# microsoft/Sora

Hardware: NVIDIA B200
Metric: 802.11a RX PHY Msamples/s (IQ in, bits out) (higher is better)
Workload: dtype int16 (fixed point; uint8 path metrics)

## Files before the change

sora_b200/csrc/fixed.cuh:

```cuda
#pragma once
#include <stdint.h>
#include <cuda_runtime.h>

namespace sb {

struct cs16 { int re, im; };

__host__ __device__ __forceinline__ int sx16(int v) { return (int)(short)v; }
__host__ __device__ __forceinline__ int sat16(int v) { return v > 32767 ? 32767 : (v < -32768 ? -32768 : v); }
__host__ __device__ __forceinline__ int wadd(int a, int b) { return (int)((unsigned)a + (unsigned)b); }

__host__ __device__ __forceinline__ cs16 unpack(uint32_t w) { cs16 c; c.re = (int)(short)(w & 0xFFFF); c.im = (int)w >> 16; return c; }
__host__ __device__ __forceinline__ uint32_t pack(cs16 c) { return ((uint32_t)c.re & 0xFFFFu) | ((uint32_t)c.im << 16); }
__host__ __device__ __forceinline__ cs16 mk(int re, int im) { cs16 c; c.re = re; c.im = im; return c; }

__host__ __device__ __forceinline__ cs16 sra(cs16 a, int n) { return mk(a.re >> n, a.im >> n); }
__host__ __device__ __forceinline__ cs16 adds(cs16 a, cs16 b) { return mk(sat16(a.re + b.re), sat16(a.im + b.im)); }
__host__ __device__ __forceinline__ cs16 subs(cs16 a, cs16 b) { return mk(sat16(a.re - b.re), sat16(a.im - b.im)); }
__host__ __device__ __forceinline__ cs16 subw(cs16 a, cs16 b) { return mk(sx16(a.re - b.re), sx16(a.im - b.im)); }
__host__ __device__ __forceinline__ cs16 cnot(cs16 a) { return mk(~a.re, ~a.im); }
__host__ __device__ __forceinline__ int neg16(int v) { return sx16(-v); }

__host__ __device__ __forceinline__ void cmul_conj32(int& re, int& im, cs16 a, cs16 b) {
    re = wadd(a.re * b.re, a.im * b.im);
    im = wadd(neg16(b.im) * a.re, b.re * a.im);
}
__host__ __device__ __forceinline__ void cmul32(int& re, int& im, cs16 a, cs16 b) {
    re = wadd(a.re * b.re, a.im * neg16(b.im));
    im = wadd(a.re * b.im, a.im * b.re);
}
__host__ __device__ __forceinline__ cs16 cmul_q15(cs16 a, cs16 b) {
    int re, im; cmul32(re, im, a, b); return mk(sx16(re >> 15), sx16(im >> 15));
}
__host__ __device__ __forceinline__ cs16 cmul_tw(cs16 a, cs16 w) {
    int re = wadd(a.re * w.re, a.im * (int)(short)~w.im);
    int im = wadd(a.re * w.im, a.im * w.re);
    return mk(sx16(re >> 15), sx16(im >> 15));
}
__host__ __device__ __forceinline__ cs16 mulj(cs16 a) { return mk(~a.im, a.re); }

__host__ __device__ __forceinline__ void r4_butterfly(cs16& a, cs16& b, cs16& c, cs16& d, cs16 w1, cs16 w2, cs16 w3) {
    a = sra(a, 2); b = sra(b, 2); c = sra(c, 2); d = sra(d, 2);
    cs16 ac = adds(a, c), bd = adds(b, d), a_c = subs(a, c), b_d = subs(b, d);
    cs16 jbd = mulj(b_d);
    a = adds(ac, bd);
    b = cmul_tw(subs(ac, bd), w2);
    c = cmul_tw(subs(a_c, jbd), w1);
    d = cmul_tw(adds(a_c, jbd), w3);
}
__host__ __device__ __forceinline__ void dft4(cs16& v0, cs16& v1, cs16& v2, cs16& v3) {
    cs16 x0 = sra(v0, 2), x1 = sra(v1, 2), x2 = sra(v2, 2), x3 = sra(v3, 2);
    cs16 s0 = adds(x0, x2), s1 = adds(x1, x3), s2 = adds(cnot(x2), x0), s3 = adds(cnot(x3), x1);
    cs16 t3 = mk(s3.im, ~s3.re);
    v0 = adds(s0, s1); v1 = adds(cnot(s1), s0); v2 = adds(s2, t3); v3 = adds(cnot(t3), s2);
}

}
```

sora_b200/csrc/rx11a_kernels.cuh:

```cuda
#pragma once
#include "tables.cuh"
#include "viterbi_k7_common.cuh"

namespace sb {

__device__ __forceinline__ int d_uatan2(const DevTables& T, int y, int x) {
    unsigned ay = y > 0 ? (unsigned)y : 0u - (unsigned)y, ax = x > 0 ? (unsigned)x : 0u - (unsigned)x;
    int ys = ay > 1 ? 31 - __clz(ay) : 0, xs = ax > 1 ? 31 - __clz(ax) : 0;
    int shift = max(xs, ys) - 6;
    if (shift > 0) { y >>= shift; x >>= shift; }
    return (int)__ldg(&T.atan2_lut[((unsigned)y & 0xFF) * 256 + ((unsigned)x & 0xFF)]);
}
__device__ __forceinline__ cs16 d_rot(const DevTables& T, int th) {
    return unpack(__ldg(T.rot + ((unsigned)th & 0xFFFFu)));
}

struct CcaState {
    uint32_t his[4][4];
    int acr[4], aci[4], eng[4];
    int his_idx, acc_i, acr_reg, aci_reg, eng_reg;
    unsigned auto_count, sense_count, high_count; int sync_state, peak_corr, peak_index;
    unsigned dc_cnt; int dc_sum_re, dc_sum_im;
    __device__ void reset() {
        for (int i = 0; i < 4; i++) { for (int j = 0; j < 4; j++) his[i][j] = 0; acr[i] = aci[i] = eng[i] = 0; }
// ... 113 lines not shown
        r4_butterfly(a, b, c, d, unpack(__ldg(T.tw64 + lane)), unpack(__ldg(T.tw64 + 16 + lane)), unpack(__ldg(T.tw64 + 32 + lane)));
        x[lane] = pack(a); x[lane + 16] = pack(b); x[lane + 32] = pack(c); x[lane + 48] = pack(d);
    }
    __syncwarp();
    if (lane < 16) {
        int base = (lane >> 2) * 16, fidx = lane & 3;
        cs16 a = unpack(x[base + fidx]), b = unpack(x[base + fidx + 4]), c = unpack(x[base + fidx + 8]), d = unpack(x[base + fidx + 12]);
        r4_butterfly(a, b, c, d, unpack(__ldg(T.tw16 + fidx)), unpack(__ldg(T.tw16 + 4 + fidx)), unpack(__ldg(T.tw16 + 8 + fidx)));
        x[base + fidx] = pack(a); x[base + fidx + 4] = pack(b); x[base + fidx + 8] = pack(c); x[base + fidx + 12] = pack(d);
    }
    __syncwarp();
    if (lane < 16) {
        cs16 a = unpack(x[4 * lane]), b = unpack(x[4 * lane + 1]), c = unpack(x[4 * lane + 2]), d = unpack(x[4 * lane + 3]);
        dft4(a, b, c, d);
        x[4 * lane] = pack(a); x[4 * lane + 1] = pack(b); x[4 * lane + 2] = pack(c); x[4 * lane + 3] = pack(d);
    }
    __syncwarp();
}
__device__ __forceinline__ int bitrev6(int i) { return (int)(__brev((unsigned)i) >> 26); }

__device__ __forceinline__ uint32_t warp_viterbi_signal(const uint8_t* soft, int lane) {
    const unsigned FULL = 0xFFFFFFFFu;
    const int cA = ((lane >> 1) ^ (lane >> 2) ^ (lane >> 4)) & 1;
    const int cB = (lane ^ (lane >> 1) ^ (lane >> 2)) & 1;
    int m0 = lane == 0 ? 0x00 : 0x30, m1 = 0x30;
    uint32_t decE[24], decO[24];
#pragma unroll
    for (int t = 0; t < 24; t++) {
        int tA = 2 * soft[2 * t], tB = 2 * soft[2 * t + 1];
        int alpha = (cA ? 14 - tA : tA) + (cB ? 14 - tB : tB), beta = 28 - alpha;
        int n0 = min((m0 + alpha) & 0xFE, ((m1 + beta) & 0xFF) | 1);
        int n1 = min((m0 + beta) & 0xFE, ((m1 + alpha) & 0xFF) | 1);
        decE[t] = __ballot_sync(FULL, n0 & 1); decO[t] = __ballot_sync(FULL, n1 & 1);
        int w = n0 | (n1 << 8);
        int wa = __shfl_sync(FULL, w, lane >> 1), wb = __shfl_sync(FULL, w, 16 + (lane >> 1));
        int sh = 8 * (lane & 1);
        m0 = (wa >> sh) & 0xFF; m1 = (wb >> sh) & 0xFF;
        if (((t + 1) & 7) == 0) {
            int mn = __reduce_min_sync(FULL, min(m0, m1)) & 0xFE;
            m0 = (m0 - mn) & 0xFF; m1 = (m1 - mn) & 0xFF;
        }
    }
    unsigned key = min(((unsigned)m0 << 8) | ((unsigned)lane << 2), ((unsigned)m1 << 8) | ((unsigned)(lane + 32) << 2));
    key = __reduce_min_sync(FULL, key);
    int pos = (int)(key >> 2) & 0x7F;
    uint32_t word = 0;
#pragma unroll
    for (int i = 0; i < 24; i++) {
        word |= (uint32_t)((pos >> 6) & 1) << (23 - i);
        pos = (pos >> 1) & 0x3F;
        int col = 23 - i;
        int bit = 0;
        if (col >= 1) { uint32_t wsel = (pos & 1) ? decO[col - 1] : decE[col - 1]; bit = (wsel >> (pos >> 1)) & 1; }
        pos |= bit << 6;
    }
    return word >> 6;
}

struct FrontTaps {
    uint32_t* freq_coeffs; uint32_t* chan_coeffs; uint32_t* fft_out; uint32_t* equalized; uint32_t* tracked; uint32_t max_sym;
    uint32_t hdr_only;
};

__device__ __forceinline__ int data_index(int bin) {
    if (bin >= 38) { if (bin == 43 || bin == 57) return -1; return bin - 38 - (bin > 43) - (bin > 57); }
    if (bin >= 1 && bin <= 26) { if (bin == 7 || bin == 21) return -1; return 24 + bin - 1 - (bin > 7) - (bin > 21); }
    return -1;
}

#define SB_FRONT_WARPS 4
#ifndef SB_FRONT_MINB
#define SB_FRONT_MINB 6
#endif
template <int STAGE>
__global__ void __launch_bounds__(32 * SB_FRONT_WARPS, SB_FRONT_MINB) k_front11a(const uint32_t* __restrict__ iq, const uint64_t* __restrict__ off,
        const uint32_t* __restrict__ len, uint32_t nframes, DevTables T, FrameInfo* __restrict__ info,
        uint8_t* __restrict__ soft_out, uint64_t soft_stride, const uint16_t* __restrict__ inv_deint, FrontTaps taps, uint32_t sh, uint32_t lsh) {
    __shared__ uint32_t s_fft[SB_FRONT_WARPS][2][64];
    __shared__ __align__(16) uint8_t s_soft[SB_FRONT_WARPS][288];
    __shared__ uint32_t s_demap[256];
    __shared__ uint8_t s_pilot[128];
    __shared__ __align__(16) uint32_t s_stage[STAGE == 2 ? SB_FRONT_WARPS : 1][2][STAGE == 2 ? 328 : 4];
    __shared__ __align__(8) unsigned long long s_mbar[STAGE == 2 ? SB_FRONT_WARPS : 1][2];
    const unsigned FULL = 0xFFFFFFFFu;
    const int lane = threadIdx.x & 31, wib = threadIdx.x >> 5;
    if (STAGE == 2 && lane == 0) {
        asm volatile("mbarrier.init.shared::cta.b64 [%0], 1;" :: "r"((uint32_t)__cvta_generic_to_shared(&s_mbar[wib][0])));
        asm volatile("mbarrier.init.shared::cta.b64 [%0], 1;" :: "r"((uint32_t)__cvta_generic_to_shared(&s_mbar[wib][1])));
        asm volatile("fence.mbarrier_init.release.cluster;" ::: "memory");
    }
    for (int i = threadIdx.x; i < 256; i += blockDim.x)
        s_demap[i] = (uint32_t)__ldg(T.demap + i) | ((uint32_t)__ldg(T.demap + 256 + i) << 8) | ((uint32_t)__ldg(T.demap + 512 + i) << 16) | ((uint32_t)__ldg(T.demap + 768 + i) << 24);
    for (int i = threadIdx.x; i < 128; i += blockDim.x) s_pilot[i] = __ldg(T.pilot_neg + i);
    __syncthreads();
    const uint32_t f = blockIdx.x * SB_FRONT_WARPS + wib;
    if (f >= nframes) return;
    FrameInfo fi = info[f];
    if (fi.status != E_SUCCESS) return;
    uint8_t* sb = s_soft[wib];
    const uint32_t* x = iq + off[f];
    const uint32_t nvec = ((len[f] << lsh) / 28u) * 28u / 8u;
    const uint32_t s0 = fi.detect_vec * 4u;
    if (fi.detect_vec + 36u > nvec) { if (lane == 0) info[f].status = E_NO_FRAME; return; }
    const int half = lane >> 4, hl = lane & 15;
    const int b0 = lane, b1 = lane + 32;
    const int r0 = bitrev6(b0), r1 = bitrev6(b1);
// ... 174 lines not shown
            const uint32_t mb = (uint32_t)__cvta_generic_to_shared(&s_mbar[wib][b]), dst = (uint32_t)__cvta_generic_to_shared(&s_stage[wib][b][0]);
            asm volatile("mbarrier.arrive.expect_tx.shared::cta.b64 _, [%0], %1;" :: "r"(mb), "r"(bytes) : "memory");
            asm volatile("cp.async.bulk.shared::cluster.global.mbarrier::complete_tx::bytes [%0], [%1], %2, [%3];" :: "r"(dst), "l"(a0), "r"(bytes), "r"(mb) : "memory");
        }
    };
    auto stage_wait = [&](int b) {
        if (st_cnt[b] == 0) return;
        const uint32_t mb = (uint32_t)__cvta_generic_to_shared(&s_mbar[wib][b]); uint32_t ok = 0;
        while (!ok) asm volatile("{ .reg .pred p; mbarrier.try_wait.parity.shared::cta.b64 p, [%1], %2; selp.u32 %0, 1, 0, p; }" : "=r"(ok) : "r"(mb), "r"(st_par[b]) : "memory");
        st_par[b] ^= 1u;
    };
    auto stage_load4 = [&](int b, uint32_t first, cs16 (&v)[4]) {
        const uint32_t skew = (uint32_t)(((uintptr_t)(x + (st_base[b] << sh)) & 15u) >> 2);
#pragma unroll
        for (int j = 0; j < 4; j++) v[j] = cmul_q15(sra(unpack(s_stage[wib][b][skew + ((first - st_base[b] + hl + 16u * j) << sh)]), 1), fcv[j]);
    };
    if (STAGE == 2 && more) stage_issue(0, s0 + 144u + 80u, 160u);
    if (STAGE == 1 && more) prefetch_regs(s0 + 144u + 80u * (1u + (uint32_t)half) + 8u);
    for (uint32_t sym = 1; more; sym += 2) {
        const bool haveA = sym_ready(sym), haveB = remain >= 2 && sym_ready(sym + 1);
        if (!haveA) { status = E_NO_FRAME; break; }
        {   cs16 v[4];
            const uint32_t mine = (half && haveB) ? sym + 1 : sym;
            const uint32_t first = s0 + 144u + 80u * mine + 8u;
            if (STAGE == 2) {
                const int b = (int)(st_i & 1u);
                const bool staged = st_base[b] == s0 + 144u + 80u * sym && st_cnt[b] >= (mine - sym + 1u) * 80u;
                stage_wait(b);
                if (staged) stage_load4(b, first, v); else load4(first, v);
                __syncwarp();
                st_i++; stage_issue((int)(st_i & 1u), s0 + 144u + 80u * (sym + 2u), 160u);
            } else if (STAGE == 1) {
                if (raw_first == first) {
#pragma unroll
                    for (int j = 0; j < 4; j++) v[j] = cmul_q15(sra(unpack(raw[j]), 1), fcv[j]);
                } else load4(first, v);
                prefetch_regs(s0 + 144u + 80u * (sym + 2u + (uint32_t)half) + 8u);
            } else load4(first, v);
            fft_from_regs(v[0], v[1], v[2], v[3]); }
        more = post_fft(0, sym);
        if (!more) break;
        if (!haveB) {
            if (remain >= 1 && !sym_ready(sym + 1)) { status = E_NO_FRAME; break; }
            sym -= 1;
            if (STAGE == 2) { stage_wait((int)(st_i & 1u)); __syncwarp(); stage_issue((int)(st_i & 1u), s0 + 144u + 80u * (sym + 2u), 160u); }
            continue;
        }
        more = post_fft(1, sym + 1);
    }
    if (STAGE == 2) { stage_wait((int)(st_i & 1u)); __syncwarp(); }
    if (lane == 0) { fi.status = status; fi.soft_bytes = soft_bytes; info[f] = fi; }
}

__host__ __device__ inline uint32_t resampled_len_40(uint32_t len44) {
    const uint32_t n = len44 / 28u * 28u, q = n / 11u, rem = n % 11u;
    const uint32_t m = 10u * q + (rem >= 1u ? 1u : 0u) + (rem > 2u ? rem - 2u : 0u);
    return m / 28u * 28u;
}
__global__ void __launch_bounds__(256) k_resample_44_40(const uint32_t* __restrict__ iq, const uint64_t* __restrict__ off, const uint32_t* __restrict__ len,
                                                        uint32_t nframes, uint32_t* __restrict__ out, uint64_t out_stride ,
                                                        uint64_t* __restrict__ off40, uint32_t* __restrict__ len40) {
    const uint32_t f = blockIdx.x;
    if (f >= nframes) return;
    const uint32_t n40 = resampled_len_40(len[f]);
    if (blockIdx.y == 0 && threadIdx.x == 0) { off40[f] = (uint64_t)f * out_stride; len40[f] = n40; }
    const uint32_t* x = iq + off[f];
    uint32_t* y = out + (size_t)f * out_stride;
    for (uint32_t m = blockIdx.y * blockDim.x + threadIdx.x; m < n40; m += gridDim.y * blockDim.x) {
        const uint32_t k = m / 10u, r = m - 10u * k;
        if (r == 0) { y[m] = __ldg(x + 11u * k); continue; }
        const int R = r == 1 ? 115 : r == 2 ? 102 : r == 3 ? 90 : r == 4 ? 77 : r == 5 ? 64 : r == 6 ? 51 : r == 7 ? 38 : r == 8 ? 26 : 13;
        const int L = r == 1 ? 13 : r == 2 ? 26 : r == 3 ? 38 : r == 4 ? 51 : r == 5 ? 64 : r == 6 ? 77 : r == 7 ? 90 : r == 8 ? 102 : 115;
        const cs16 a = unpack(__ldg(x + 11u * k + r)), b = unpack(__ldg(x + 11u * k + r + 1u));
        y[m] = pack(mk(sx16((a.re * R + b.re * L) >> 7), sx16((a.im * R + b.im * L) >> 7)));
    }
}

}
```

sora_b200/csrc/sb200.cu:

```cuda
#include "../../include/sora_b200.h"
#include "viterbi_k7_re.cuh"
#include "viterbi_k7_lane.cuh"
#include "rx11b_kernels.cuh"
#include "rx11n_kernels.cuh"
#include "tx11a_kernels.cuh"
#include "tx11b_kernels.cuh"
#include "tx11b_legacy_kernels.cuh"
#include "tx11n_kernels.cuh"
#include "fir_kernels.cuh"
#include <stdlib.h>
#include <string>
#include <vector>
#include <chrono>
#include <string.h>
#include <new>
#include <stdio.h>
#include <thread>
#include <mutex>
#include <condition_variable>
#include <atomic>
#include <emmintrin.h>

using namespace sb;

// ... 293 lines not shown
            if (r[1]) return h->fail(SB200_E_INVALID, "slot exceeds iq_total_samples");
            h->tab_max_len = r[0]; h->tab_host = need_host_copy;
            if (h->tab_immutable) { h->tab_off = frame_off; h->tab_len = frame_len; h->tab_n = nframes; h->tab_total = iq_total; }
        }
        *d_off = frame_off; *d_len = frame_len; *max_len = h->tab_max_len; *host_valid = h->tab_host && (cached || need_host_copy);
        return SB200_OK;
    }
    h->tab_off = nullptr;
    offh.resize(nframes); lenh.resize(nframes);
    if (off_dev) CK(cudaMemcpyAsync(offh.data(), frame_off, nframes * 8ull, cudaMemcpyDeviceToHost, st)); else memcpy(offh.data(), frame_off, nframes * 8ull);
    if (len_dev) CK(cudaMemcpyAsync(lenh.data(), frame_len, nframes * 4ull, cudaMemcpyDeviceToHost, st)); else memcpy(lenh.data(), frame_len, nframes * 4ull);
    if (off_dev || len_dev) CK(cudaStreamSynchronize(st));
    uint32_t mx = 0;
    for (uint32_t i = 0; i < nframes; i++) {
        if (lenh[i] > iq_total || offh[i] > iq_total - lenh[i]) return h->fail(SB200_E_INVALID, "slot exceeds iq_total_samples");
        if (lenh[i] > mx) mx = lenh[i];
    }
    if (off_dev) *d_off = frame_off; else { CK(h->off.need(nframes * 8ull)); CK(cudaMemcpyAsync(h->off.p, offh.data(), nframes * 8ull, cudaMemcpyHostToDevice, st)); *d_off = (const uint64_t*)h->off.p; }
    if (len_dev) *d_len = frame_len; else { CK(h->len.need(nframes * 4ull)); CK(cudaMemcpyAsync(h->len.p, lenh.data(), nframes * 4ull, cudaMemcpyHostToDevice, st)); *d_len = (const uint32_t*)h->len.p; }
    *max_len = mx; *host_valid = true;
    return SB200_OK;
}

static cudaError_t vring_need(sb200_handle* h, uint32_t n) {
    if (n >= h->lane_min) return h->vring.need((size_t)((n + SB_VL_FR - 1) / SB_VL_FR) * SB_VL_NB8D * SB_VL_ENTRY * 16);
    return cudaSuccess;
}
template <int CR>
static void launch_viterbi_re(sb200_handle* h, uint32_t n, cudaStream_t s, const uint8_t* soft, uint64_t soft_stride, const uint32_t* list, const uint32_t* cnt,
                              const FrameInfo* info, const VitJob& job, uint8_t* out, uint64_t out_stride, uint32_t raw_off, uint32_t* nraw) {
    const unsigned g = (n + SB_VR_FR - 1) / SB_VR_FR, gp = (n + 15) / 16;
    uint4* const ring = (uint4*)h->vring.p;
    h->last_vit = n >= h->lane_min ? "k_viterbi_lane" : "k_viterbi_re";
    if (n >= h->lane_min && h->vl_hb == 8 && h->vl_defer) k_viterbi_lane<CR, 8, true><<<(n + SB_VL_FR - 1) / SB_VL_FR, 32, h->vl_pad_smem, s>>>(soft, soft_stride, n, list, cnt, info, job, out, out_stride, raw_off, nraw, ring, h->vl_flags);
    else if (n >= h->lane_min && h->vl_hb == 8) k_viterbi_lane<CR, 8><<<(n + SB_VL_FR - 1) / SB_VL_FR, 32, h->vl_pad_smem, s>>>(soft, soft_stride, n, list, cnt, info, job, out, out_stride, raw_off, nraw, ring, h->vl_flags);
    else if (n >= h->lane_min)       k_viterbi_lane<CR, 6><<<(n + SB_VL_FR - 1) / SB_VL_FR, 32, h->vl_pad_smem, s>>>(soft, soft_stride, n, list, cnt, info, job, out, out_stride, raw_off, nraw, ring, h->vl_flags);
    else if (h->use_pair)            k_viterbi_re<CR, 1><<<gp, 32, 0, s>>>(soft, soft_stride, n, list, cnt, info, job, out, out_stride, raw_off, nraw);
    else                             k_viterbi_re<CR, 2><<<g, 32, 0, s>>>(soft, soft_stride, n, list, cnt, info, job, out, out_stride, raw_off, nraw);
}

static int launch_chunk(sb200_handle* h, const uint32_t* iq_base, const uint64_t* d_off, const uint32_t* d_len, uint32_t f0, uint32_t f1,
                        uint64_t soft_stride, uint64_t row, cudaStream_t sf, cudaStream_t sv, cudaEvent_t front_done, FrontTaps taps, bool timed, const int2* dc_init = nullptr, uint32_t chunk_idx = 0, uint32_t sh = 1, uint32_t lsh = 0) {
    const uint32_t n = f1 - f0;
    FrameInfo* d_info = (FrameInfo*)h->info.p + f0;
    uint8_t* d_soft = (uint8_t*)h->soft.p + (size_t)f0 * soft_stride;
    uint8_t* d_out = (uint8_t*)h->out.p + (size_t)f0 * row;
    uint32_t* d_status = (uint32_t*)h->status.p + f0; uint32_t* d_crc = (uint32_t*)h->crc.p + f0;
    if (timed) CK(cudaEventRecord(h->evk[0], sf));
    k_sync11a<<<(n + 127) / 128, 128, 0, sf>>>(iq_base, d_off + f0, d_len + f0, n, h->cca_thr, h->T, d_info, dc_init ? dc_init + f0 : nullptr, sh, lsh);
    if (timed) CK(cudaEventRecord(h->evk[1], sf));
    {   const dim3 g((n + SB_FRONT_WARPS - 1) / SB_FRONT_WARPS), b(32 * SB_FRONT_WARPS);
        if (h->front_stage == 2) k_front11a<2><<<g, b, 0, sf>>>(iq_base, d_off + f0, d_len + f0, n, h->T, d_info, d_soft, soft_stride, h->inv_deint, taps, sh, lsh);
        else if (h->front_stage == 1) k_front11a<1><<<g, b, 0, sf>>>(iq_base, d_off + f0, d_len + f0, n, h->T, d_info, d_soft, soft_stride, h->inv_deint, taps, sh, lsh);
        else k_front11a<0><<<g, b, 0, sf>>>(iq_base, d_off + f0, d_len + f0, n, h->T, d_info, d_soft, soft_stride, h->inv_deint, taps, sh, lsh); }
    if (timed) CK(cudaEventRecord(h->evk[2], sf));
    if (sv != sf) { CK(cudaEventRecord(front_done, sf)); CK(cudaStreamWaitEvent(sv, front_done, 0)); }
    VitJob job{}; job.depth = 256; job.lookahead = 24; job.raw = 0;
    if (h->use_v2) {
        const unsigned g = (n + SB_VQ_FR - 1) / SB_VQ_FR, b = 32 * SB_VQ_WARPS;
        k_viterbi_quad<CR_34><<<g, b, h->vq_pad_smem, sv>>>(d_soft, soft_stride, n, d_info, job, h->T, d_out, row, d_status, d_crc);
        k_viterbi_quad<CR_12><<<g, b, 0, sv>>>(d_soft, soft_stride, n, d_info, job, h->T, d_out, row, d_status, d_crc);
        k_viterbi_quad<CR_23><<<g, b, 0, sv>>>(d_soft, soft_stride, n, d_info, job, h->T, d_out, row, d_status, d_crc);
        h->launches += 5;
    } else {
        CK(vring_need(h, n));
        uint32_t* d_list = (uint32_t*)h->vlist.p + 3 * (size_t)f0; uint32_t* d_cnt = (uint32_t*)h->vcnt.p + 4 * (size_t)chunk_idx;
        CK(cudaMemsetAsync(d_cnt, 0, 16, sv));
        k_vit_lists<<<(n + 255) / 256, 256, 0, sv>>>(d_info, n, d_cnt, d_list);
        launch_viterbi_re<CR_34>(h, n, sv, d_soft, soft_stride, d_list, d_cnt, d_info, job, d_out, row, 14u, d_status);
        launch_viterbi_re<CR_12>(h, n, sv, d_soft, soft_stride, d_list, d_cnt, d_info, job, d_out, row, 14u, d_status);
        launch_viterbi_re<CR_23>(h, n, sv, d_soft, soft_stride, d_list, d_cnt, d_info, job, d_out, row, 14u, d_status);
        k_sink11a<<<(n + 127) / 128, 128, 0, sv>>>(d_out, row, n, d_info, h->T, d_status, d_crc);
        h->launches += 7;
    }
    if (timed) CK(cudaEventRecord(h->evk[3], sv));
    return SB200_OK;
}

static int rx11a_run(sb200_handle* h, const int16_t* iq, uint64_t iq_total, const uint64_t* frame_off, const uint32_t* frame_len,
                     uint32_t nframes, uint8_t* out_bytes, uint32_t out_stride, sb200_frame_result* res, cudaStream_t st,
                     FrontTaps taps, uint8_t* soft_host, uint64_t soft_host_stride, const int2* dc_init = nullptr, bool no_chunk = false, bool rate20 = false) {
    if (!h || !iq || !frame_off || !frame_len || !res) return h ? h->fail(SB200_E_INVALID, "null argument") : SB200_E_INVALID;
    if (nframes == 0) return SB200_OK;
    CK(cudaSetDevice(h->device));
    const bool iq_dev = is_device_ptr(iq);
    std::vector<uint64_t>& offh = h->offh; std::vector<uint32_t>& lenh = h->lenh;
    const uint64_t* d_off; const uint32_t* d_len; uint32_t max_len = 0; bool tab_on_host = false;
    {
        const bool may_chunk = !no_chunk && !rate20 && !iq_dev && h->chunk_frames != 0 && nframes > h->chunk_frames;
        int rc = slot_table(h, frame_off, frame_len, nframes, iq_total, may_chunk, st, &d_off, &d_len, &max_len, &tab_on_host);
        if (rc != SB200_OK) return rc;
        if (rate20) { if (max_len > 0x7FFFFFFFu) return h->fail(SB200_E_INVALID, "slot too long"); max_len <<= 1; }
    }
    const uint64_t max_sym = (max_len / 2u) / 80u + 1u;
    const uint64_t soft_stride = ((max_sym * 288ull) + 15ull) & ~15ull;
    const uint64_t row = 2560;
    CK(h->info.need(nframes * sizeof(FrameInfo)));
    CK(h->soft.need(nframes * soft_stride));
    CK(h->out.need(nframes * row));
    CK(h->status.need(nframes * 4ull)); CK(h->crc.need(nframes * 4ull)); CK(h->res.need(nframes * sizeof(sb200_frame_result)));
    CK(h->vlist.need(nframes * 12ull));
    const bool tapping = taps.freq_coeffs || taps.fft_out || soft_host || dc_init;
    const uint32_t want = (no_chunk || rate20) ? 0u : iq_dev ? h->chunk_frames_device : h->chunk_frames;
    const uint32_t chunk = (want == 0 || tapping || nframes <= want || (!iq_dev && !tab_on_host)) ? nframes : want;
    const bool pipelined = chunk < nframes;
    CK(h->vcnt.need(16ull * ((nframes + chunk - 1) / chunk)));
    const bool res_dev_all = is_device_ptr(res), out_dev_all = out_bytes && is_device_ptr(out_bytes);
// ... 148 lines not shown
    bool host_out = false;
    if (pipelined) {
        if (out_bytes && out_stride && out_dev_all) { const size_t w = out_stride < row ? out_stride : row; CK(cudaMemcpy2DAsync(out_bytes, out_stride, h->out.p, row, w, nframes, cudaMemcpyDeviceToDevice, st)); }
        if ((out_bytes && out_stride && !out_dev_all) || !res_dev_all) CK(cudaStreamSynchronize(st));
        return SB200_OK;
    }
    if (out_bytes && out_stride) {
        const size_t w = out_stride < row ? out_stride : row;
        const bool od = is_device_ptr(out_bytes);
        CK(cudaMemcpy2DAsync(out_bytes, out_stride, h->out.p, row, w, nframes, od ? cudaMemcpyDeviceToDevice : cudaMemcpyDeviceToHost, st));
        host_out |= !od;
    }
    if (!res_dev) { CK(cudaMemcpyAsync(res, d_res, nframes * sizeof(sb200_frame_result), cudaMemcpyDeviceToHost, st)); host_out = true; }
    if (soft_host) { CK(cudaMemcpy2DAsync(soft_host, soft_host_stride, h->soft.p, soft_stride, soft_host_stride < soft_stride ? soft_host_stride : soft_stride, nframes, cudaMemcpyDeviceToHost, st)); host_out = true; }
    if (host_out) CK(cudaStreamSynchronize(st));
    return SB200_OK;
}

extern "C" void* sb200_host_alloc(size_t bytes) { void* p = nullptr; if (bytes == 0 || cudaHostAlloc(&p, bytes, cudaHostAllocPortable) != cudaSuccess) { cudaGetLastError(); return nullptr; } return p; }
extern "C" void sb200_host_free(void* p) { if (p) cudaFreeHost(p); }

extern "C" int sb200_rx11a_streams(sb200_handle* h, const int16_t* iq, uint64_t iq_total, const uint64_t* stream_off, const uint32_t* stream_len,
                                   uint32_t nstreams, uint32_t max_frames, uint8_t* out_bytes, uint32_t out_stride, sb200_frame_result* res,
                                   uint32_t* sample_index, uint32_t* nframes_out, void* cuda_stream) {
    if (!h || !iq || !stream_off || !stream_len || !res || !nframes_out) return h ? h->fail(SB200_E_INVALID, "null argument") : SB200_E_INVALID;
    cudaStream_t st = (cudaStream_t)cuda_stream;
    CK(cudaSetDevice(h->device));
    if (is_device_ptr(res) || (out_bytes && is_device_ptr(out_bytes)) || is_device_ptr(stream_off) || is_device_ptr(stream_len) || is_device_ptr(nframes_out))
        return h->fail(SB200_E_INVALID, "stream mode takes its tables and returns its results in host memory");
    for (uint32_t s = 0; s < nstreams; s++) { nframes_out[s] = 0; if (stream_off[s] + stream_len[s] > iq_total) return h->fail(SB200_E_INVALID, "capture exceeds iq_total_samples"); }
    if (nstreams == 0 || max_frames == 0) return SB200_OK;
    const int16_t* d_iq = iq;
    if (!is_device_ptr(iq)) {
        CK(h->iq.need(iq_total * 4ull));
        for (uint32_t s = 0; s < nstreams; s++) if (stream_len[s]) CK(cudaMemcpyAsync((char*)h->iq.p + stream_off[s] * 4ull, iq + 2ull * stream_off[s], stream_len[s] * 4ull, cudaMemcpyHostToDevice, st));
        d_iq = (const int16_t*)h->iq.p;
    }
    const uint32_t n = nstreams;
    const bool trace = getenv("SB200_TRACE") != nullptr; const auto t_begin = std::chrono::steady_clock::now();
    std::vector<uint64_t> off0(n); std::vector<uint32_t> len0(n);
    for (uint32_t s = 0; s < n; s++) { off0[s] = stream_off[s]; len0[s] = stream_len[s] >= 28u ? stream_len[s] : 0u; }
    CK(h->soff.need(n * 8ull)); CK(h->slen.need(n * 4ull)); CK(h->dcbuf.need(n * sizeof(int2))); CK(h->spos.need(n * 4ull)); CK(h->snev.need(n * 4ull + 64));
    CK(h->sev.need((size_t)n * max_frames * sizeof(StreamEvent))); CK(h->info.need(n * sizeof(FrameInfo)));
    CK(cudaMemcpyAsync(h->soff.p, off0.data(), n * 8ull, cudaMemcpyHostToDevice, st)); CK(cudaMemcpyAsync(h->slen.p, len0.data(), n * 4ull, cudaMemcpyHostToDevice, st));
    CK(cudaMemsetAsync(h->dcbuf.p, 0, n * sizeof(int2), st)); CK(cudaMemsetAsync(h->spos.p, 0, n * 4ull, st)); CK(cudaMemsetAsync(h->snev.p, 0, n * 4ull + 64, st));
    uint32_t* d_live = (uint32_t*)h->snev.p + n;
    FrontTaps hdr{}; hdr.hdr_only = 1;
    const uint32_t ROUND = 8;
    for (uint32_t done_passes = 0; done_passes < max_frames;) {
        CK(cudaMemsetAsync(d_live, 0, ROUND * 4ull, st));
        uint32_t k = 0;
        for (; k < ROUND && done_passes + k < max_frames; k++) {
            k_sync11a<<<(n + 127) / 128, 128, 0, st>>>((const uint32_t*)d_iq, (const uint64_t*)h->soff.p, (const uint32_t*)h->slen.p, n, h->cca_thr, h->T, (FrameInfo*)h->info.p, (const int2*)h->dcbuf.p, 1u, 0u);
            k_front11a<0><<<(n + SB_FRONT_WARPS - 1) / SB_FRONT_WARPS, 32 * SB_FRONT_WARPS, 0, st>>>((const uint32_t*)d_iq, (const uint64_t*)h->soff.p, (const uint32_t*)h->slen.p, n, h->T, (FrameInfo*)h->info.p, nullptr, 0, h->inv_deint, hdr, 1u, 0u);
            k_stream_advance<<<(n + 127) / 128, 128, 0, st>>>((const FrameInfo*)h->info.p, n, (uint64_t*)h->soff.p, (uint32_t*)h->slen.p, (int2*)h->dcbuf.p, (uint32_t*)h->spos.p, (uint32_t*)h->snev.p, max_frames, (StreamEvent*)h->sev.p, d_live + k);
            h->launches += 3;
        }
        CK(cudaGetLastError());
        uint32_t live[16]; CK(cudaMemcpyAsync(live, d_live, ROUND * 4ull, cudaMemcpyDeviceToHost, st)); CK(cudaStreamSynchronize(st));
        done_passes += k;
        if (live[k - 1] == 0) break;
    }
    const auto t_scout = std::chrono::steady_clock::now();
    std::vector<uint32_t> nev(n); CK(cudaMemcpy(nev.data(), h->snev.p, n * 4ull, cudaMemcpyDeviceToHost));
    size_t E = 0; for (uint32_t s = 0; s < n; s++) E += nev[s];
    if (E == 0) return SB200_OK;
    std::vector<StreamEvent> ev((size_t)n * max_frames);
    CK(cudaMemcpy(ev.data(), h->sev.p, ev.size() * sizeof(StreamEvent), cudaMemcpyDeviceToHost));
    std::vector<uint64_t> off(E); std::vector<uint32_t> len(E); std::vector<int2> dcv(E); std::vector<sb200_frame_result> r(E);
    const uint32_t row = out_bytes ? (out_stride < 2560u ? out_stride : 2560u) : 0u;
    std::vector<uint8_t> bytes((size_t)E * row);
    {   size_t e = 0;
        for (uint32_t s = 0; s < n; s++) for (uint32_t j = 0; j < nev[s]; j++, e++) { const StreamEvent& v = ev[(size_t)s * max_frames + j]; off[e] = v.off; len[e] = v.len; dcv[e] = v.dc; } }
    CK(h->dcbuf.need(E * sizeof(int2))); CK(cudaMemcpyAsync(h->dcbuf.p, dcv.data(), E * sizeof(int2), cudaMemcpyHostToDevice, st));
    FrontTaps taps{};
    int rc = rx11a_run(h, d_iq, iq_total, off.data(), len.data(), (uint32_t)E, row ? bytes.data() : nullptr, row, r.data(), st, taps, nullptr, 0, (const int2*)h->dcbuf.p, true);
    if (rc != SB200_OK) return rc;
    {   size_t e = 0;
        for (uint32_t s = 0; s < n; s++) {
            for (uint32_t j = 0; j < nev[s]; j++, e++) {
                const size_t slot = (size_t)s * max_frames + j;
                if (r[e].status == SB200_FRAME_NONE) return h->fail(SB200_E_CUDA, "internal: stream scout and batch decode disagree about a frame");
                res[slot] = r[e];
                if (sample_index) sample_index[slot] = ev[slot].pos_after;
                if (row) memcpy(out_bytes + slot * out_stride, bytes.data() + e * row, row);
            }
            nframes_out[s] = nev[s];
        } }
    if (trace) { const auto t_end = std::chrono::steady_clock::now();
        fprintf(stderr, "[sb200] rx11a_streams: %u captures, %zu events, %llu samples: scout %.3f ms, batch %.3f ms\n", n, E, (unsigned long long)iq_total,
                std::chrono::duration<double, std::milli>(t_scout - t_begin).count(), std::chrono::duration<double, std::milli>(t_end - t_scout).count()); }
    return rc;
}

extern "C" int sb200_rx11a_stream(sb200_handle* h, const int16_t* iq, uint64_t nsamples, uint32_t max_frames, uint8_t* out_bytes, uint32_t out_stride,
                                  sb200_frame_result* res, uint32_t* sample_index, uint32_t* nframes_out, void* cuda_stream) {
    if (!h || !nframes_out) return h ? h->fail(SB200_E_INVALID, "null argument") : SB200_E_INVALID;
    if (nsamples > 0xFFFFFF00ull) return h->fail(SB200_E_INVALID, "capture longer than 2^32 samples: split it");
    const uint64_t off = 0; const uint32_t len = (uint32_t)nsamples;
    return sb200_rx11a_streams(h, iq, nsamples, &off, &len, 1, max_frames, out_bytes, out_stride, res, sample_index, nframes_out, cuda_stream);
}

static const int16_t kHalfBand31[31] = {-121, 0, 209, 0, -381, 0, 644, 0, -1056, 0, 1759, 0, -3278, 0, 10391, 16434, 10391, 0, -3278, 0, 1759, 0, -1056, 0, 644, 0, -381, 0, 209, 0, -121};
extern "C" int sb200_fir_decimate2(sb200_handle* h, const int16_t* iq, uint64_t n_in, const int16_t* taps, uint32_t ntaps, int16_t* out, void* cuda_stream) {
    if (!h || !iq || !out) return h ? h->fail(SB200_E_INVALID, "null argument") : SB200_E_INVALID;
    if (!taps) { taps = kHalfBand31; ntaps = 31; }
    if ((ntaps & 1u) == 0 || ntaps > SB_FIR_MAXTAPS) return h->fail(SB200_E_INVALID, "ntaps must be odd and at most 63");
// ... 765 lines not shown
```

Baseline: 96550.

## Add direct front-end kernel with wrapping FFT butterflies and register-resident signal Viterbi

Adds k_front11a_direct, a new OFDM front-end kernel used by default (stage 0) and in the stream-scouting loop. It swaps the saturating add/sub in the radix-4 FFT butterflies for plain wrapping integer adds, keeps the SIGNAL-field Viterbi survivor bits in lane registers fetched by shuffle, and simplifies the per-symbol loop to load two symbols per warp half with no staged prefetch. The aim is fewer instructions per FFT and less shared-memory use. Dropping saturation can change fixed-point results if intermediates overflow, and losing the prefetch pipeline may expose load latency.

```diff
diff --git a/sora_b200/csrc/fixed.cuh b/sora_b200/csrc/fixed.cuh
--- a/sora_b200/csrc/fixed.cuh
+++ b/sora_b200/csrc/fixed.cuh
@@ -48,11 +48,28 @@
     c = cmul_tw(subs(a_c, jbd), w1);
     d = cmul_tw(adds(a_c, jbd), w3);
 }
+__host__ __device__ __forceinline__ void r4_butterfly_i16(cs16& a, cs16& b, cs16& c, cs16& d, cs16 w1, cs16 w2, cs16 w3) {
+    a = sra(a, 2); b = sra(b, 2); c = sra(c, 2); d = sra(d, 2);
+    const cs16 ac = mk(a.re + c.re, a.im + c.im), bd = mk(b.re + d.re, b.im + d.im);
+    const cs16 a_c = mk(a.re - c.re, a.im - c.im), jbd = mulj(mk(b.re - d.re, b.im - d.im));
+    a = mk(ac.re + bd.re, ac.im + bd.im);
+    b = cmul_tw(mk(ac.re - bd.re, ac.im - bd.im), w2);
+    c = cmul_tw(mk(a_c.re - jbd.re, a_c.im - jbd.im), w1);
+    d = cmul_tw(mk(a_c.re + jbd.re, a_c.im + jbd.im), w3);
+}
 __host__ __device__ __forceinline__ void dft4(cs16& v0, cs16& v1, cs16& v2, cs16& v3) {
     cs16 x0 = sra(v0, 2), x1 = sra(v1, 2), x2 = sra(v2, 2), x3 = sra(v3, 2);
     cs16 s0 = adds(x0, x2), s1 = adds(x1, x3), s2 = adds(cnot(x2), x0), s3 = adds(cnot(x3), x1);
     cs16 t3 = mk(s3.im, ~s3.re);
     v0 = adds(s0, s1); v1 = adds(cnot(s1), s0); v2 = adds(s2, t3); v3 = adds(cnot(t3), s2);
 }
+__host__ __device__ __forceinline__ void dft4_i16(cs16& v0, cs16& v1, cs16& v2, cs16& v3) {
+    const cs16 x0 = sra(v0, 2), x1 = sra(v1, 2), x2 = sra(v2, 2), x3 = sra(v3, 2);
+    const cs16 s0 = mk(x0.re + x2.re, x0.im + x2.im), s1 = mk(x1.re + x3.re, x1.im + x3.im);
+    const cs16 s2 = mk(~x2.re + x0.re, ~x2.im + x0.im), s3 = mk(~x3.re + x1.re, ~x3.im + x1.im);
+    const cs16 t3 = mk(s3.im, ~s3.re);
+    v0 = mk(s0.re + s1.re, s0.im + s1.im); v1 = mk(~s1.re + s0.re, ~s1.im + s0.im);
+    v2 = mk(s2.re + t3.re, s2.im + t3.im); v3 = mk(~t3.re + s2.re, ~t3.im + s2.im);
+}
 
 }
diff --git a/sora_b200/csrc/rx11a_kernels.cuh b/sora_b200/csrc/rx11a_kernels.cuh
--- a/sora_b200/csrc/rx11a_kernels.cuh
+++ b/sora_b200/csrc/rx11a_kernels.cuh
@@ -189,6 +189,45 @@
         int col = 23 - i;
         int bit = 0;
         if (col >= 1) { uint32_t wsel = (pos & 1) ? decO[col - 1] : decE[col - 1]; bit = (wsel >> (pos >> 1)) & 1; }
+        pos |= bit << 6;
+    }
+    return word >> 6;
+}
+
+__device__ __forceinline__ uint32_t warp_viterbi_signal_lanes(const uint8_t* soft, int lane) {
+    const unsigned FULL = 0xFFFFFFFFu;
+    const int cA = ((lane >> 1) ^ (lane >> 2) ^ (lane >> 4)) & 1;
+    const int cB = (lane ^ (lane >> 1) ^ (lane >> 2)) & 1;
+    int m0 = lane == 0 ? 0x00 : 0x30, m1 = 0x30;
+    uint32_t myE = 0, myO = 0;
+#pragma unroll
+    for (int t = 0; t < 24; t++) {
+        int tA = 2 * soft[2 * t], tB = 2 * soft[2 * t + 1];
+        int alpha = (cA ? 14 - tA : tA) + (cB ? 14 - tB : tB), beta = 28 - alpha;
+        int n0 = min((m0 + alpha) & 0xFE, ((m1 + beta) & 0xFF) | 1);
+        int n1 = min((m0 + beta) & 0xFE, ((m1 + alpha) & 0xFF) | 1);
+        const uint32_t e = __ballot_sync(FULL, n0 & 1), o = __ballot_sync(FULL, n1 & 1);
+        myE = lane == t ? e : myE; myO = lane == t ? o : myO;
+        int w = n0 | (n1 << 8);
+        int wa = __shfl_sync(FULL, w, lane >> 1), wb = __shfl_sync(FULL, w, 16 + (lane >> 1));
+        int sh = 8 * (lane & 1);
+        m0 = (wa >> sh) & 0xFF; m1 = (wb >> sh) & 0xFF;
+        if (((t + 1) & 7) == 0) {
+            int mn = __reduce_min_sync(FULL, min(m0, m1)) & 0xFE;
+            m0 = (m0 - mn) & 0xFF; m1 = (m1 - mn) & 0xFF;
+        }
+    }
+    unsigned key = min(((unsigned)m0 << 8) | ((unsigned)lane << 2), ((unsigned)m1 << 8) | ((unsigned)(lane + 32) << 2));
+    key = __reduce_min_sync(FULL, key);
+    int pos = (int)(key >> 2) & 0x7F;
+    uint32_t word = 0;
+#pragma unroll
+    for (int i = 0; i < 24; i++) {
+        word |= (uint32_t)((pos >> 6) & 1) << (23 - i);
+        pos = (pos >> 1) & 0x3F;
+        int col = 23 - i;
+        int bit = 0;
+        if (col >= 1) { uint32_t wsel = __shfl_sync(FULL, (pos & 1) ? myO : myE, col - 1); bit = (wsel >> (pos >> 1)) & 1; }
         pos |= bit << 6;
     }
     return word >> 6;
@@ -469,6 +508,216 @@
     if (lane == 0) { fi.status = status; fi.soft_bytes = soft_bytes; info[f] = fi; }
 }
 
+template <int N> struct IntC { static constexpr int value = N; };
+
+__global__ void __launch_bounds__(32 * SB_FRONT_WARPS, SB_FRONT_MINB) k_front11a_direct(const uint32_t* __restrict__ iq, const uint64_t* __restrict__ off,
+        const uint32_t* __restrict__ len, uint32_t nframes, DevTables T, FrameInfo* __restrict__ info,
+        uint8_t* __restrict__ soft_out, uint64_t soft_stride, const uint16_t* __restrict__ inv_deint, FrontTaps taps, uint32_t sh, uint32_t lsh) {
+    __shared__ uint32_t s_fft[SB_FRONT_WARPS][2][64];
+    __shared__ __align__(16) uint8_t s_soft[SB_FRONT_WARPS][2][288];
+    __shared__ uint32_t s_demap[256];
+    __shared__ uint8_t s_pilot[128];
+    const unsigned FULL = 0xFFFFFFFFu;
+    const int lane = threadIdx.x & 31, wib = threadIdx.x >> 5;
+    for (int i = threadIdx.x; i < 256; i += blockDim.x)
+        s_demap[i] = (uint32_t)__ldg(T.demap + i) | ((uint32_t)__ldg(T.demap + 256 + i) << 8) | ((uint32_t)__ldg(T.demap + 512 + i) << 16) | ((uint32_t)__ldg(T.demap + 768 + i) << 24);
+    for (int i = threadIdx.x; i < 128; i += blockDim.x) s_pilot[i] = __ldg(T.pilot_neg + i);
+    __syncthreads();
+    const uint32_t f = blockIdx.x * SB_FRONT_WARPS + wib;
+    if (f >= nframes) return;
+    FrameInfo fi = info[f];
+    if (fi.status != E_SUCCESS) return;
+    const uint32_t* x = iq + off[f];
+    const uint32_t nvec = ((len[f] << lsh) / 28u) * 28u / 8u;
+    const uint32_t s0 = fi.detect_vec * 4u;
+    if (fi.detect_vec + 36u > nvec) { if (lane == 0) info[f].status = E_NO_FRAME; return; }
+    const int half = lane >> 4, hl = lane & 15;
+    const int b0 = lane, b1 = lane + 32;
+    const int r0 = bitrev6(b0), r1 = bitrev6(b1);
+    const cs16 w64_1 = unpack(__ldg(T.tw64 + hl)), w64_2 = unpack(__ldg(T.tw64 + 16 + hl)), w64_3 = unpack(__ldg(T.tw64 + 32 + hl));
+    const cs16 w16_1 = unpack(__ldg(T.tw16 + (hl & 3))), w16_2 = unpack(__ldg(T.tw16 + 4 + (hl & 3))), w16_3 = unpack(__ldg(T.tw16 + 8 + (hl & 3)));
+    auto fft_from_regs = [&](cs16 a, cs16 b, cs16 c, cs16 d) {
+        uint32_t* xb = s_fft[wib][half];
+        r4_butterfly_i16(a, b, c, d, w64_1, w64_2, w64_3);
+        xb[hl] = pack(a); xb[hl + 16] = pack(b); xb[hl + 32] = pack(c); xb[hl + 48] = pack(d);
+        __syncwarp();
+        {   const int base = (hl >> 2) * 16 + (hl & 3);
+            cs16 p = unpack(xb[base]), q = unpack(xb[base + 4]), r = unpack(xb[base + 8]), t = unpack(xb[base + 12]);
+            r4_butterfly_i16(p, q, r, t, w16_1, w16_2, w16_3);
+            xb[base] = pack(p); xb[base + 4] = pack(q); xb[base + 8] = pack(r); xb[base + 12] = pack(t); }
+        __syncwarp();
+        {   cs16 p = unpack(xb[4 * hl]), q = unpack(xb[4 * hl + 1]), r = unpack(xb[4 * hl + 2]), t = unpack(xb[4 * hl + 3]);
+            dft4_i16(p, q, r, t);
+            xb[4 * hl] = pack(p); xb[4 * hl + 1] = pack(q); xb[4 * hl + 2] = pack(r); xb[4 * hl + 3] = pack(t); }
+        __syncwarp();
+    };
+    {
+        cs16 l0 = sra(unpack(__ldg(x + ((s0 + 8u + b0) << sh))), 1), l1 = sra(unpack(__ldg(x + ((s0 + 8u + b1) << sh))), 1);
+        cs16 h0 = unpack(__ldg(x + ((s0 + 72u + b0) << sh))), h1 = unpack(__ldg(x + ((s0 + 72u + b1) << sh)));
+        int re0, im0, re1, im1; cmul_conj32(re0, im0, h0, l0); cmul_conj32(re1, im1, h1, l1);
+        int sr = wadd(re0 >> 5, re1 >> 5), si = wadd(im0 >> 5, im1 >> 5);
+        for (int o = 16; o; o >>= 1) { sr = wadd(sr, __shfl_xor_sync(FULL, sr, o)); si = wadd(si, __shfl_xor_sync(FULL, si, o)); }
+        fi.cfo_est = (int)(short)(((uint32_t)d_uatan2(T, si, sr)) / 64u);
+    }
+    cs16 fcv[4];
+#pragma unroll
+    for (int j = 0; j < 4; j++) fcv[j] = d_rot(T, fi.cfo_est * (hl + 16 * j));
+    auto load4 = [&](uint32_t first, cs16 (&v)[4]) {
+#pragma unroll
+        for (int j = 0; j < 4; j++) v[j] = cmul_q15(sra(unpack(__ldg(x + ((first + hl + 16u * j) << sh))), 1), fcv[j]);
+    };
+    {   cs16 v[4]; load4(s0 + 8u, v); fft_from_regs(v[0], v[1], v[2], v[3]); }
+    cs16 ch0, ch1;
+    {
+        const uint32_t* xb = s_fft[wib][0];
+        auto inv = [&](cs16 y, int bin) -> cs16 {
+            if (bin >= 28 && bin <= 35) return mk(0, 0);
+            int e = wadd(y.re * y.re, y.im * y.im) >> 8;
+            int L = __ldg(T.lts_pos + bin) ? 1600 : -1600;
+            int re, im; cmul_conj32(re, im, mk(L, 0), y);
+            return e ? mk(sx16(re / e), sx16(im / e)) : mk(0, 0);
+        };
+        ch0 = inv(unpack(xb[r0]), b0); ch1 = inv(unpack(xb[r1]), b1);
+    }
+    __syncwarp();
+    if (taps.freq_coeffs) { taps.freq_coeffs[(size_t)f * 64 + b0] = pack(d_rot(T, fi.cfo_est * b0)); taps.freq_coeffs[(size_t)f * 64 + b1] = pack(d_rot(T, fi.cfo_est * b1));
+                            taps.chan_coeffs[(size_t)f * 64 + b0] = pack(ch0); taps.chan_coeffs[(size_t)f * 64 + b1] = pack(ch1); }
+    const int k0 = b0, k1 = b1 - 64;
+    const bool v0 = (k0 >= 1 && k0 <= 26), v1 = (k1 >= -26 && k1 <= -1);
+    const bool z0 = (b0 >= 28), z1 = (b1 <= 35);
+    const int d0 = data_index(b0), d1 = data_index(b1);
+    cs16 comp0 = mk(0x7fff, 0), comp1 = mk(0x7fff, 0);
+    int CFO_comp = 0, SFO_comp = 0, CFO_tr = 0, SFO_tr = 0; unsigned symbol_count = 127;
+    uint32_t soft_bytes = 0;
+    uint8_t* sout = soft_out + (size_t)f * soft_stride;
+    uint32_t status = E_SUCCESS;
+    uint32_t pos[6];
+    auto load_positions = [&](auto nbc) {
+        constexpr int NB = decltype(nbc)::value;
+        const uint16_t* inv = inv_deint + (NB == 1 ? 0 : NB == 2 ? 48 : NB == 4 ? 144 : 336);
+        const uint32_t base = (uint32_t)wib * (2u * 288u);
+#pragma unroll
+        for (int i = 0; i < NB; i++)
+            pos[i] = (base + (d0 >= 0 ? __ldg(inv + d0 * NB + i) : 0u)) | ((base + (d1 >= 0 ? __ldg(inv + d1 * NB + i) : 0u)) << 16);
+    };
+    auto track = [&](int h, uint32_t sym, auto nbc) {
+        constexpr int NB = decltype(nbc)::value;
+        const uint32_t* xb = s_fft[wib][h];
+        const cs16 F0 = unpack(xb[r0]), F1 = unpack(xb[r1]);
+        cs16 E0 = mk(0, 0), E1 = mk(0, 0);
+        if (!z0) { int re, im; cmul32(re, im, F0, ch0); E0 = mk(sx16(re >> 8), sx16(im >> 8)); }
+        if (!z1) { int re, im; cmul32(re, im, F1, ch1); E1 = mk(sx16(re >> 8), sx16(im >> 8)); }
+        const cs16 C0 = cmul_q15(E0, comp0), C1 = cmul_q15(E1, comp1);
+        int th = 0;
+        {
+            const bool hi = lane == 11 || lane == 25, neg = lane == 21;
+            const int py = hi ? C1.im : (neg ? -C0.im : C0.im), px = hi ? C1.re : (neg ? -C0.re : C0.re);
+            const int a = d_uatan2(T, py, px);
+            if (hi || lane == 7 || lane == 21) th = a;
+        }
+        if (s_pilot[symbol_count]) th = sx16(th + 0x8000);
+        const int th1 = __shfl_sync(FULL, th, 11), th2 = __shfl_sync(FULL, th, 25), th3 = __shfl_sync(FULL, th, 7), th4 = __shfl_sync(FULL, th, 21);
+        symbol_count++; if (symbol_count >= 127) symbol_count = 0;
+        const int avg = sx16((th1 + th2 + th3 + th4) / 4);
+        const int del = sx16(((th3 - th1) / 28 + (th4 - th2) / 28) >> 1);
+        cs16 R0 = mk(0, 0), R1 = mk(0, 0);
+        if (!z0) R0 = cmul_q15(C0, v0 ? d_rot(T, avg + k0 * del) : mk(0, 0));
+        if (!z1) R1 = cmul_q15(C1, v1 ? d_rot(T, avg + k1 * del) : mk(0, 0));
+        CFO_tr = sx16(CFO_tr + (avg >> 2)); SFO_tr = sx16(SFO_tr + (del >> 2));
+        CFO_comp = sx16(CFO_comp + avg + CFO_tr); SFO_comp = sx16(SFO_comp + del + SFO_tr);
+        if (v0) comp0 = d_rot(T, CFO_comp + k0 * SFO_comp);
+        if (v1) comp1 = d_rot(T, CFO_comp + k1 * SFO_comp);
+        if (taps.fft_out && sym < taps.max_sym) {
+            size_t o = ((size_t)f * taps.max_sym + sym) * 64;
+            taps.fft_out[o + b0] = pack(F0); taps.fft_out[o + b1] = pack(F1);
+            taps.equalized[o + b0] = pack(E0); taps.equalized[o + b1] = pack(E1);
+            taps.tracked[o + b0] = pack(R0); taps.tracked[o + b1] = pack(R1);
+        }
+        uint8_t* sb = &s_soft[0][h][0];
+        auto demap = [&](cs16 r, int d, int sh16) {
+            if (d < 0) return;
+            const unsigned re = (unsigned)min(max(r.re >> 4, -128), 127) & 0xFF, im = (unsigned)min(max(r.im >> 4, -128), 127) & 0xFF;
+            const uint32_t wr = s_demap[re], wi = s_demap[im];
+            auto at = [&](int i) -> uint8_t& { return sb[(pos[i] >> sh16) & 0xFFFFu]; };
+            if (NB == 1) { at(0) = (uint8_t)wr; }
+            else if (NB == 2) { at(0) = (uint8_t)wr; at(1) = (uint8_t)wi; }
+            else if (NB == 4) { at(0) = (uint8_t)wr; at(1) = (uint8_t)(wr >> 8); at(2) = (uint8_t)wi; at(3) = (uint8_t)(wi >> 8); }
+            else { at(0) = (uint8_t)wr; at(1) = (uint8_t)(wr >> 16); at(2) = (uint8_t)(wr >> 24);
+                   at(3) = (uint8_t)wi; at(4) = (uint8_t)(wi >> 16); at(5) = (uint8_t)(wi >> 24); }
+        };
+        demap(R0, d0, 0); demap(R1, d1, 16);
+        __syncwarp();
+    };
+    auto sym_ready = [&](uint32_t sym) { return (s0 + 144u + 80u * sym + 80u) / 4u <= nvec; };
+    auto finish = [&]() { if (lane == 0) { fi.status = status; fi.soft_bytes = soft_bytes; info[f] = fi; } };
+    if (!sym_ready(0)) { status = E_NO_FRAME; finish(); return; }
+    {   cs16 v[4]; load4(s0 + 144u + 8u, v); fft_from_regs(v[0], v[1], v[2], v[3]); }
+    load_positions(IntC<1>());
+    track(0, 0u, IntC<1>());
+    uint32_t nb = 1;
+    {
+        const uint32_t sig = warp_viterbi_signal_lanes(s_soft[wib][0], lane) & 0xFFFFFFu;
+        bool ok = !(sig & 0xFC0010u);
+        uint32_t par = (sig >> 16) ^ sig; par ^= par >> 8; par ^= par >> 4; par ^= par >> 2; par ^= par >> 1;
+        ok = ok && !(par & 1);
+        uint32_t rate = 0; int nd = 0, cr = CR_12;
+        switch (sig & 0xF) {
+            case 0xB: rate = 6000; nd = 24; nb = 1; cr = CR_12; break;   case 0xF: rate = 9000; nd = 36; nb = 1; cr = CR_34; break;
+            case 0xA: rate = 12000; nd = 48; nb = 2; cr = CR_12; break;  case 0xE: rate = 18000; nd = 72; nb = 2; cr = CR_34; break;
+            case 0x9: rate = 24000; nd = 96; nb = 4; cr = CR_12; break;  case 0xD: rate = 36000; nd = 144; nb = 4; cr = CR_34; break;
+            case 0x8: rate = 48000; nd = 192; nb = 6; cr = CR_23; break; case 0xC: rate = 54000; nd = 216; nb = 6; cr = CR_34; break;
+            default: if (ok) fi.rate_kbps = 0; ok = false;
+        }
+        const uint32_t L = (sig >> 5) & 0xFFF;
+        if (ok && rate) { fi.rate_kbps = rate; fi.code_rate = cr; }
+        if (ok) { fi.length = L; ok = L <= 2500; }
+        if (!ok) { status = E_PLCP_HEADER_FAIL; finish(); return; }
+        fi.nsym_total = (L * 8 + 16 + 6 + nd - 1) / nd + 1;
+        fi.ncbps = 48 * nb;
+    }
+    if (taps.hdr_only) {
+        if (!sym_ready(fi.nsym_total - 1u)) status = E_NO_FRAME;
+        finish(); return;
+    }
+    const uint32_t need = fi.nsym_total - 1u;
+    const uint64_t sym_max = (4ull * nvec + 3ull - (s0 + 224u)) / 80u;
+    const uint32_t ndata = (uint32_t)min((uint64_t)need, sym_max);
+    if (ndata < need) status = E_NO_FRAME;
+    const bool wide = ((((uintptr_t)sout) | (uintptr_t)soft_stride) & 15u) == 0;
+    auto data_loop = [&](auto nbc) {
+        constexpr int NB = decltype(nbc)::value, NCBPS = 48 * NB;
+        load_positions(nbc);
+        auto emit = [&](int h) {
+            if (wide) {
+                const uint4* src = (const uint4*)s_soft[wib][h]; uint4* dst = (uint4*)(sout + soft_bytes);
+                if (lane < NCBPS / 16) dst[lane] = src[lane];
+            } else {
+                const uint32_t* src = (const uint32_t*)s_soft[wib][h]; uint32_t* dst = (uint32_t*)(sout + soft_bytes);
+#pragma unroll
+                for (int w = lane; w < NCBPS / 4; w += 32) dst[w] = src[w];
+            }
+            soft_bytes += NCBPS;
+        };
+        uint32_t sym = 1;
+        for (uint32_t p = ndata >> 1; p; p--, sym += 2) {
+            {   cs16 v[4]; load4(s0 + 144u + 80u * (sym + (uint32_t)half) + 8u, v); fft_from_regs(v[0], v[1], v[2], v[3]); }
+            track(0, sym, nbc); emit(0);
+            track(1, sym + 1u, nbc); emit(1);
+        }
+        if (ndata & 1u) {
+            {   cs16 v[4]; load4(s0 + 144u + 80u * sym + 8u, v); fft_from_regs(v[0], v[1], v[2], v[3]); }
+            track(0, sym, nbc); emit(0);
+        }
+    };
+    switch (nb) {
+        case 1: data_loop(IntC<1>()); break;
+        case 2: data_loop(IntC<2>()); break;
+        case 4: data_loop(IntC<4>()); break;
+        default: data_loop(IntC<6>()); break;
+    }
+    finish();
+}
+
 __host__ __device__ inline uint32_t resampled_len_40(uint32_t len44) {
     const uint32_t n = len44 / 28u * 28u, q = n / 11u, rem = n % 11u;
     const uint32_t m = 10u * q + (rem >= 1u ? 1u : 0u) + (rem > 2u ? rem - 2u : 0u);
diff --git a/sora_b200/csrc/sb200.cu b/sora_b200/csrc/sb200.cu
--- a/sora_b200/csrc/sb200.cu
+++ b/sora_b200/csrc/sb200.cu
@@ -369,7 +369,7 @@
     {   const dim3 g((n + SB_FRONT_WARPS - 1) / SB_FRONT_WARPS), b(32 * SB_FRONT_WARPS);
         if (h->front_stage == 2) k_front11a<2><<<g, b, 0, sf>>>(iq_base, d_off + f0, d_len + f0, n, h->T, d_info, d_soft, soft_stride, h->inv_deint, taps, sh, lsh);
         else if (h->front_stage == 1) k_front11a<1><<<g, b, 0, sf>>>(iq_base, d_off + f0, d_len + f0, n, h->T, d_info, d_soft, soft_stride, h->inv_deint, taps, sh, lsh);
-        else k_front11a<0><<<g, b, 0, sf>>>(iq_base, d_off + f0, d_len + f0, n, h->T, d_info, d_soft, soft_stride, h->inv_deint, taps, sh, lsh); }
+        else k_front11a_direct<<<g, b, 0, sf>>>(iq_base, d_off + f0, d_len + f0, n, h->T, d_info, d_soft, soft_stride, h->inv_deint, taps, sh, lsh); }
     if (timed) CK(cudaEventRecord(h->evk[2], sf));
     if (sv != sf) { CK(cudaEventRecord(front_done, sf)); CK(cudaStreamWaitEvent(sv, front_done, 0)); }
     VitJob job{}; job.depth = 256; job.lookahead = 24; job.raw = 0;
@@ -624,7 +624,7 @@
         uint32_t k = 0;
         for (; k < ROUND && done_passes + k < max_frames; k++) {
             k_sync11a<<<(n + 127) / 128, 128, 0, st>>>((const uint32_t*)d_iq, (const uint64_t*)h->soff.p, (const uint32_t*)h->slen.p, n, h->cca_thr, h->T, (FrameInfo*)h->info.p, (const int2*)h->dcbuf.p, 1u, 0u);
-            k_front11a<0><<<(n + SB_FRONT_WARPS - 1) / SB_FRONT_WARPS, 32 * SB_FRONT_WARPS, 0, st>>>((const uint32_t*)d_iq, (const uint64_t*)h->soff.p, (const uint32_t*)h->slen.p, n, h->T, (FrameInfo*)h->info.p, nullptr, 0, h->inv_deint, hdr, 1u, 0u);
+            k_front11a_direct<<<(n + SB_FRONT_WARPS - 1) / SB_FRONT_WARPS, 32 * SB_FRONT_WARPS, 0, st>>>((const uint32_t*)d_iq, (const uint64_t*)h->soff.p, (const uint32_t*)h->slen.p, n, h->T, (FrameInfo*)h->info.p, nullptr, 0, h->inv_deint, hdr, 1u, 0u);
             k_stream_advance<<<(n + 127) / 128, 128, 0, st>>>((const FrameInfo*)h->info.p, n, (uint64_t*)h->soff.p, (uint32_t*)h->slen.p, (int2*)h->dcbuf.p, (uint32_t*)h->spos.p, (uint32_t*)h->snev.p, max_frames, (StreamEvent*)h->sev.p, d_live + k);
             h->launches += 3;
         }
```

New measurement: 100,700, median of 6. +4.3%, better.
